# beer-asr/beer

Measured on AMD Instinct MI355X. Metric: frames/sec per VB iteration (E+M), higher is better.
Workload: dtype f32

## Files before the change

beer_amd/_hip.py:

```python

import ctypes
import os
import threading

import torch

_HERE = os.path.dirname(os.path.abspath(__file__))
LIB_PATH = os.environ.get('BEER_HIP_LIB') or os.path.join(_HERE, 'csrc', 'libbeer_hip.so')

F32, F64, I16 = 0, 1, 2
FULL, DIAG, ISO = 0, 1, 2
SEG = 8
MAX_HUBS = 4
COV_CODE = {'full': FULL, 'diagonal': DIAG, 'isotropic': ISO}
EINVAL = -100000


class HipUnavailable(RuntimeError):
    'Raised when the HIP extension or the GPU is missing (no CPU fallback).'


class HipError(RuntimeError):
    rc = None

# ... 274 lines not shown
    'beer_ng_from_natural': _from,
    'beer_ing_expected_stats': _four, 'beer_ing_log_norm': _four, 'beer_ing_natural': _four,
    'beer_ing_from_natural': _from,
    'beer_dirichlet_expected_stats': _dir, 'beer_dirichlet_log_norm': _dir,
    'beer_dirichlet_natural': _dir, 'beer_dirichlet_from_natural': _dir,
    'beer_dirichlet_log_weights': _dir,
    'beer_sb_transform_stats': [c_i, c_i, c_p, c_p, c_p, c_p],
    'beer_sb_log_weights': [c_i, c_i, c_p, c_p, c_p, c_p, c_p],
    'beer_sb_set_log_weights': [c_i, c_i, c_i, c_p, c_p, c_p, c_p],
    'beer_sb_set_transform_stats': [c_i, c_i, c_i, c_p, c_p, c_p, c_p],
    'beer_gamma_expected_stats': _gam, 'beer_gamma_log_norm': _gam,
    'beer_gamma_natural': _gam,
    'beer_gamma_from_natural': [c_i, c_i, c_p, c_p, c_p, c_p],
    'beer_kl_div': [c_i, c_i, c_i, c_p, c_p, c_p, c_p, c_p, c_p, c_p],
    'beer_natural_grad_step': [c_i, c_l, c_p, c_p, c_p, c_d, c_p, c_p],
    'beer_suffstats_expand': [c_i, c_i, c_l, c_i, c_p, c_p, c_p],
    'beer_mixtureset_estep': [c_i, c_i, c_l, c_i, c_i, c_i, c_p, c_p, c_p, c_p, c_d,
                              c_p, c_p, c_p, c_p, c_p, c_z, c_p],
    'beer_normal_accumulate': [c_i, c_i, c_l, c_i, c_i, c_i, c_p, c_p, c_p, c_p, c_p, c_z,
                               c_p],
    'beer_mixture_estep_packed': [c_i, c_l, c_i, c_i, c_p, c_p, c_p, c_p, c_p, c_p, c_p, c_z,
                                  c_p],
    'beer_normal_accumulate_packed': [c_i, c_l, c_i, c_i, c_p, c_p, c_p, c_p, c_z, c_p],
    'beer_mixtureset_estep_packed': [c_i, c_l, c_i, c_i, c_i, c_p, c_p, c_p, c_p, c_p, c_p, c_p,
                                     c_z, c_p],
    'beer_mixtureset_accumulate_packed': [c_i, c_l, c_i, c_i, c_i, c_p, c_p, c_p, c_p, c_p, c_z,
                                          c_p],
    'beer_unpack_resps': [c_l, c_i, c_p, c_p, c_p],
    'beer_mixtureset_accumulate_fused': [c_i, c_l, c_i, c_i, c_i, c_p, c_p, c_p, c_p, c_p, c_p,
                                         c_p, c_p, c_z, c_p],
# ... 286 lines not shown
```

beer_amd/csrc/estep_bf16.hip:

```cpp

#include <cstdlib>
#include <type_traits>
#include <utility>

#include "estep_mfma.h"
#include "estep_tiles.h"

namespace beer_mfma {

namespace {

typedef __bf16 bf8 __attribute__((ext_vector_type(8)));
typedef unsigned int u4 __attribute__((ext_vector_type(4)));
typedef float f32x2 __attribute__((ext_vector_type(2)));

template <int V> using ic = std::integral_constant<int, V>;
template <int... I, typename F>
__device__ __forceinline__ void static_for_impl(std::integer_sequence<int, I...>, F&& f) {
    (f(ic<I>{}), ...);
}
template <int N, typename F>
__device__ __forceinline__ void static_for(F&& f) {
    static_for_impl(std::make_integer_sequence<int, N>{}, static_cast<F&&>(f));
}
// ... 62 lines not shown
    const int a = t & 0xff, b = ((t >> 8) & 0xff) + e, sq = t >> 16;
    if (a == Dp && b - e == Dp) {
        *is_const = true;
        return 0.0;
    }
    if (k >= K) return 0.0;
    if (sq) return b < D ? -0.5 * (double)row[cov == BEER_ISO ? D : D + b] : 0.0;
    if (a < D) {
        if (b >= D || b < a) return 0.0;
        return b == a ? -0.5 * (double)row[D + a * D + a]
                      : -0.5 * ((double)row[D + a * D + b] + (double)row[D + b * D + a]);
    }
    return b < D ? (double)row[b] : 0.0;
}

__global__ __launch_bounds__(256) void const_max_kernel(int cov, int D, int K,
                                                        const float* __restrict__ E,
                                                        const float* __restrict__ logw,
                                                        float* __restrict__ c0) {
    __shared__ double red[8];
    const int Q = stats_dim(cov, D);
    double m = -1.0e300;
    for (int k = threadIdx.x; k < K; k += blockDim.x) {
        const double v = const_total(cov, D, E + (size_t)k * Q, logw ? (double)logw[k] : 0.0);
        if (v == v && v > m && v < 1.0e300) m = v;
    }
    m = block_max(m, red);
    if (threadIdx.x == 0) c0[0] = m > -1.0e300 ? (float)m : 0.f;
}

__global__ __launch_bounds__(256) void packx_kernel(int cov, int D, int K, int NT,
                                                    const float* __restrict__ E,
                                                    const float* __restrict__ logw,
                                                    unsigned short* __restrict__ P,
                                                    int* __restrict__ tab, int G, int Gp,
                                                    const float* __restrict__ c0, int lane_major) {
    extern __shared__ __attribute__((aligned(16))) char pack_lds[];
    const int nk = nk16_of(cov, D), nent = nk * 32;
    const int slot = blockIdx.x;
    const int k = slot % Gp < G ? (slot / Gp) * G + slot % Gp : K;
    const int chunk = slot / (NT * 16), kk = slot % (NT * 16);
    const int c = lane_major ? kk % NT : 4 * (kk / 64) + (kk % 4);
    const int i = lane_major ? kk / NT : (kk % 64) / 4;
    if (slot == 0)
        for (int s = threadIdx.x; s < (nk + 1) * 8; s += blockDim.x) tab[s] = slabx_entry(cov, D, s);
    const int Qs = stats_dim(cov, D);
    float* rowl = reinterpret_cast<float*>(pack_lds);
    if (k < K)
        for (int q = threadIdx.x; q < Qs; q += blockDim.x) rowl[q] = E[(size_t)k * Qs + q];
    __syncthreads();
    unsigned short* base = P + ((size_t)chunk * nk * NT) * (NP * 512);
    auto put = [&](int q, float v) {
// ... 2 lines not shown
        unsigned short p[3];
        split3_scalar(v, p);
        dst[0] = p[0];
        dst[512] = p[1];
        dst[1024] = p[2];
    };
    const int nslab = nslabx_of(cov, D);
    for (int q = threadIdx.x; q < nent; q += blockDim.x) {
        bool is_const;
        const double v = entry_value(cov, D, K, k, q / 4, q % 4, rowl, &is_const);
        if (!is_const) {
            put(q, (float)v);
        } else if (q % 4 == 0) {
            const bool last = q / 4 == nslab - 1;
            const double want = k < K ? const_share(cov, D, q / 4, rowl, logw ? (double)logw[k] : 0.0) -
                                            (last ? (double)c0[0] : 0.0)
                                      : (last ? kPadLogit : 0.0);
            const float hi = (float)want;
            const double rem = (want - (double)hi) * (1.0 / (double)kConstEps);
            put(q, hi);
            put(q + 1, (rem == rem && fabs(rem) < 1.0e30) ? (float)rem : 0.f);
            put(q + 2, 0.f);
            put(q + 3, 0.f);
        }
    }
}

inline int xcd_chunk_group(int ny, size_t chunk_bytes) {
    int cg = (int)((size_t)(2 << 20) / (chunk_bytes ? chunk_bytes : 1));
    return cg < 1 ? 1 : (cg > ny ? ny : cg);
}
// ... 1799 lines not shown
    const int Kreal = S * G, nk = nk16_of(cov, D);
    LlhxArgs a = {};
    a.nframes = nframes, a.D = D, a.K = S * f.Gp, a.S = S, a.G = f.Gp;
    a.gl = f.gl, a.jw = f.jw, a.nchunks = f.nchunks, a.nk = nk;
    a.nku = (nslabx_of(cov, D) + 7) / 8;
    a.X = X, a.resps = resps, a.log_norm = log_norm, a.llh_sum = llh_sum, a.img = image, a.s = s;
    const PtabLayout l = ptab_layout(f.nchunks, nk, f.NT);
    int* tab = reinterpret_cast<int*>(reinterpret_cast<char*>(ws) + l.tab);
    float* c0 = reinterpret_cast<float*>(reinterpret_cast<char*>(ws) + l.c0);
    a.P = ws, a.tab = tab, a.c0 = c0;
    if (f.xt) {
        a.xt_out = reinterpret_cast<float*>(reinterpret_cast<char*>(resps) +
                                            packed_tiles_bytes(nframes, a.K));
        a.xt_floats = xt_pieces(D) * (kPiece / 4);
    }
    hipLaunchKernelGGL(const_max_kernel, dim3(1), dim3(256), 0, s, cov, D, Kreal, expT, logw, c0);
    hipLaunchKernelGGL(packx_kernel, dim3(f.nchunks * f.NT * 16), dim3(256),
                       (size_t)stats_dim(cov, D) * sizeof(float), s, cov, D, Kreal, f.NT, expT, logw,
                       reinterpret_cast<unsigned short*>(ws), tab, G, f.Gp, c0,
                       f.lane_major ? 1 : 0);
    BEER_LAUNCH_CHECK();
    const int nku = f.lnfi ? f.nku : 0, gq = f.lnfi ? f.lnfi_g : f.GQ;
    for (const LlhxRow& r : kLlhxRows)
        if (r.NT == f.NT && r.GQ == gq && r.nku == nku && r.packed == f.packed && r.lno == f.lno &&
            r.img == f.img && r.bl == f.bl) {
            const auto launch = cov == BEER_FULL ? r.full : r.sq;
            return launch ? launch(a) : BEER_EINVAL;
        }
    return BEER_EINVAL;
}

// ... 87 lines not shown
    BEER_LAUNCH_CHECK();
    return BEER_OK;
}

}

int acc_bf16x3_packed(int cov, int64_t nframes, int D, int K, const float* X, const void* Rimg,
                      double* acc, void* ws, size_t ws_bytes, hipStream_t s, int S, int G,
                      const float* SR) {
    const AccxForm f = accx_form(cov, D, K, S, G, SR != nullptr);
    const AccxLayout l = accx_layout(cov, nframes, D, K, S, G, SR != nullptr);
    if (f.rc != BEER_OK || ws_bytes < l.bytes) return BEER_EINVAL;
    char* w = reinterpret_cast<char*>(ws);
    double* Sp = reinterpret_cast<double*>(w + l.Sp);
    int* tab = reinterpret_cast<int*>(w + l.tab);
    hipError_t e = hipMemsetAsync(Sp, 0, (size_t)K * f.nslab * 4 * sizeof(double), s);
    if (e != hipSuccess) return -(int)e;
    hipLaunchKernelGGL(tabx_kernel, dim3(1), dim3(256), 0, s, cov, D, f.nslab, tab);
    BEER_LAUNCH_CHECK();
    const int64_t tiles = (nframes + kAxFT - 1) / kAxFT;
    const float* Xt;
    if (f.xt_reused) {
        Xt = reinterpret_cast<const float*>(reinterpret_cast<const char*>(Rimg) +
                                            packed_tiles_bytes(nframes, K));
    } else {
        float* image = reinterpret_cast<float*>(w + l.Xt);
        hipLaunchKernelGGL(xt_image_kernel, dim3((unsigned)tiles), dim3(256), 0, s, nframes, D, f.NX,
                           X, image);
        BEER_LAUNCH_CHECK();
        Xt = image;
    }
    float* Gt = nullptr;
    if (f.sr) {
// ... 155 lines not shown
                     const float* sr, const void* image, double* acc, void* ws, size_t ws_bytes,
                     hipStream_t s) {
    const AccfForm f = accf_form(cov, D, S, G, image != nullptr);
    const AccfLayout l = accf_layout(cov, D, S, G);
    if (f.rc != BEER_OK || ws_bytes < l.bytes) return BEER_EINVAL;
    const int Kreal = S * G, K = S * f.Gp, NTC = f.NTC, nk = nk16_of(cov, D);
    const int nchunks = f.nchunks, kpad = nchunks * NTC * 16;
    const int nslab = nslab_of(cov, D), nq = nslab * 4;
    char* w = reinterpret_cast<char*>(ws);
    void* P = w + l.P;
    int* tab = reinterpret_cast<int*>(w + l.tab);
    float* c0 = reinterpret_cast<float*>(w + l.c0);
    double* Sp = reinterpret_cast<double*>(w + l.Sp);
    hipError_t e = hipMemsetAsync(Sp, 0, (size_t)Kreal * nq * sizeof(double), s);
    if (e != hipSuccess) return -(int)e;
    hipLaunchKernelGGL(const_max_kernel, dim3(1), dim3(256), 0, s, cov, D, Kreal, expT, logw, c0);
    hipLaunchKernelGGL(packx_kernel, dim3(kpad), dim3(256),
                       (size_t)stats_dim(cov, D) * sizeof(float), s, cov, D, Kreal, NTC, expT, logw,
                       reinterpret_cast<unsigned short*>(P), tab, G, f.Gp, c0, 0);
    BEER_LAUNCH_CHECK();
    const int waves = f.waves;
    const int rounds = beer::option(BEER_OPT_ACCF_ROUNDS);
    int64_t gz = ((waves == 8 ? 256 : 512) * rounds + nchunks - 1) / nchunks;
    gz = (gz + 7) / 8 * 8;
    const int64_t chain = nframes >= ((int64_t)4 << 20) ? kAfMaxFramesPerWave : kAfMaxFramesPerWave / 2;
    const int64_t min_z = (nframes + (int64_t)waves * chain - 1) / ((int64_t)waves * chain);
    const int64_t max_z = (nframes + 32 * waves - 1) / (32 * waves);
    if (gz > max_z) gz = max_z;
    if (gz < min_z) gz = min_z;
    if (gz < 1) gz = 1;
    const FrameSplit z = frame_split(nframes, gz, 32 * waves);
// ... 27 lines not shown
```

beer_amd/csrc/estep_tiles.h:

```cpp
#pragma once
#include <type_traits>

#include <hip/hip_runtime.h>

#include "common.h"

namespace beer_mfma {

using namespace beer;

typedef float f32x4 __attribute__((ext_vector_type(4)));
typedef double f64x4 __attribute__((ext_vector_type(4)));

template <typename T> struct Mma;
template <> struct Mma<float> {
    using acc_t = f32x4;
    using vec4_t = f32x4;
    static __device__ __forceinline__ acc_t mma(float a, float b, acc_t c) {
        return __builtin_amdgcn_mfma_f32_16x16x4f32(a, b, c, 0, 0, 0);
    }
    static __device__ __forceinline__ int row(int g, int r) { return 4 * g + r; }
    static __device__ __forceinline__ float exp_neg(float x) {
        return __builtin_amdgcn_exp2f(x * 1.44269504088896340736f);
    }
// ... 233 lines not shown
        acc[idx] += v;
    }
}
__global__ void unpack_kernel(int cov, int D, int K, const double* __restrict__ Sp,
                              double* __restrict__ acc) {
    unpack_stats<false>(cov, D, K, Sp, acc);
}
__global__ void unpackx_kernel(int cov, int D, int K, const double* __restrict__ Sp,
                               double* __restrict__ acc) {
    unpack_stats<true>(cov, D, K, Sp, acc);
}
__global__ void tabx_kernel(int cov, int D, int n, int* __restrict__ tab) {
    for (int s = blockIdx.x * blockDim.x + threadIdx.x; s < n; s += gridDim.x * blockDim.x)
        tab[s] = slabx_entry(cov, D, s);
}

}

constexpr int kPackedFrames = 64, kPackedComps = 128, kPackedPieces = 3;
constexpr int kPackedPlaneWords = kPackedComps * kPackedFrames / 2;

__host__ __device__ inline size_t packed_word(int64_t tau, int nblk, int beta, int kk, int f6) {
    const int half = kk * kPackedFrames + (((f6 >> 3) ^ (kk & 7)) << 3) + (f6 & 7);
    return ((size_t)tau * nblk + beta) * (kPackedPieces * kPackedPlaneWords) + (half >> 1);
}

__device__ __forceinline__ unsigned cvt_pk_bf16(float a, float b) {
    typedef __bf16 bf2_t __attribute__((ext_vector_type(2)));
    typedef float f2_t __attribute__((ext_vector_type(2)));
    const f2_t v = {a, b};
// ... 312 lines not shown
```

beer_amd/csrc/expfam.hip:

```cpp

#include "common.h"

using namespace beer;

namespace {

constexpr int kNwThreads = 1024;
inline int nw_threads(int K, int D) {
    return K <= 512 && D >= 16 ? 1024 : 256;
}
constexpr int kMaxFullDim = 128;




template <typename T>
__global__ __launch_bounds__(kNwThreads) void nw_expected_stats_kernel(
    int D, const T* __restrict__ mean, const T* __restrict__ scale,
    const T* __restrict__ W, const T* __restrict__ dof, T* __restrict__ out,
    T* __restrict__ lnorm) {
    extern __shared__ __attribute__((aligned(16))) char smem[];
    double* A = reinterpret_cast<double*>(smem);
    double* m = A + D * D;
    double* pm = m + D;
// ... 386 lines not shown
template <typename T>
__global__ __launch_bounds__(64) void kl_kernel(int Q, const T* es, const T* eq,
                                                const T* ep, const T* lq,
                                                const T* lp, T* out) {
    const int k = blockIdx.x;
    double s = 0.0;
    for (int i = threadIdx.x; i < Q; i += 64) {
        const size_t j = (size_t)k * Q + i;
        s += (double)es[j] * ((double)ep[j] - (double)eq[j]);
    }
    s = wave_sum(s);
    if (threadIdx.x == 0) out[k] = (T)((double)lp[k] - (double)lq[k] - s);
}

template <typename T>
__global__ void nat_grad_kernel(int64_t n, const T* ep, const T* eq, const T* st,
                                double lr, T* out) {
    const int64_t i = (int64_t)blockIdx.x * blockDim.x + threadIdx.x;
    if (i >= n) return;
    const double q = (double)eq[i];
    out[i] = (T)(q + lr * ((double)ep[i] + (double)st[i] - q));
}

template <typename T>
__global__ void suffstats_kernel(int cov, int64_t T_, int D, const T* X, T* out) {
    const int Q = stats_dim(cov, D);
    const int64_t total = T_ * Q;
    for (int64_t idx = (int64_t)blockIdx.x * blockDim.x + threadIdx.x; idx < total;
         idx += (int64_t)gridDim.x * blockDim.x) {
        const int64_t t = idx / Q;
        const int q = (int)(idx % Q);
        const T* x = X + t * D;
        T v;
        if (q < D) {
            v = x[q];
        } else if (q >= Q - 2) {
// ... 149 lines not shown
    return BEER_OK;
}

template <typename T>
int nat_grad_launch(int64_t n, const void* ep, const void* eq, const void* st, double lr,
                    void* out, void* stream) {
    BEER_REQUIRE(n >= 0);
    if (n == 0) return BEER_OK;
    hipLaunchKernelGGL(nat_grad_kernel<T>, dim3(blocks_for(n, 256)), dim3(256), 0,
                       as_stream(stream), n, (const T*)ep, (const T*)eq, (const T*)st, lr, (T*)out);
    BEER_LAUNCH_CHECK();
    return BEER_OK;
}

template <typename T>
int suffstats_launch(int cov, int64_t T_, int D, const void* X, void* out, void* stream) {
    BEER_REQUIRE(T_ >= 0 && D >= 1 && cov >= 0 && cov <= 2);
    if (T_ == 0) return BEER_OK;
    const int64_t total = T_ * stats_dim(cov, D);
    const int blocks = (int)((total + 255) / 256 > 65536 ? 65536 : (total + 255) / 256);
    hipLaunchKernelGGL(suffstats_kernel<T>, dim3(blocks), dim3(256), 0, as_stream(stream), cov, T_,
                       D, (const T*)X, (T*)out);
    BEER_LAUNCH_CHECK();
    return BEER_OK;
}

}


namespace {
// ... 292 lines not shown
}
int beer_gamma_log_norm(int dtype, int n, const void* shape, const void* rate, void* out, void* stream) {
    BEER_DISPATCH(dtype, gamma_launch, 3, n, shape, rate, out, nullptr, stream);
}

int beer_kl_div(int dtype, int K, int Q, const void* es, const void* eq, const void* ep,
                const void* lq, const void* lp, void* out, void* stream) {
    BEER_DISPATCH(dtype, kl_launch, K, Q, es, eq, ep, lq, lp, out, stream);
}

int beer_natural_grad_step(int dtype, int64_t n, const void* eta_prior, const void* eta_post,
                           const void* stats, double lrate, void* out, void* stream) {
    BEER_DISPATCH(dtype, nat_grad_launch, n, eta_prior, eta_post, stats, lrate, out, stream);
}

int beer_suffstats_expand(int dtype, int cov, int64_t T, int D, const void* X, void* out,
                          void* stream) {
    BEER_DISPATCH(dtype, suffstats_launch, cov, T, D, X, out, stream);
}

}
```

beer_amd/dists/families.py:

```python

import math

import torch

from .. import _hip
from ..stats import FrameStats, reference_layout_enabled
from .expfam import ConjugateLikelihood, ExponentialFamily, make_std_params

__all__ = [
    'NormalLikelihood', 'NormalWishart', 'NormalWishartStdParams',
    'NormalDiagonalLikelihood', 'NormalGamma', 'NormalGammaStdParams',
    'IsotropicNormalLikelihood', 'IsotropicNormalGamma',
    'IsotropicNormalGammaStdParams',
    'CategoricalLikelihood', 'Dirichlet', 'DirichletStdParams',
    'GammaLikelihood', 'Gamma', 'GammaStdParams',
]


def _run(name, dtype, ints, ins, outs):
    code = _hip.dtype_code(dtype)
    dins = [_hip.on_device(t, dtype) for t in ins]
    _hip.call(name, code, *ints, *[_hip.ptr(t) for t in dins], *[_hip.ptr(t) for t in outs])


# ... 352 lines not shown
    def log_weights(self):
        return self._memoised('logw', lambda: self._launch('beer_dirichlet_log_weights'))

    def log_weights64(self):
        c = self.params.concentrations
        if c.dtype == torch.float64:
            return self.log_weights()

        def compute():
            c2 = c.double().reshape(1, -1) if c.dim() <= 1 else c.double()
            out = _empty(tuple(c2.shape), c2, torch.float64)
            _run('beer_dirichlet_log_weights', torch.float64, tuple(c2.shape), (c2,), (out,))
            return out.to(c.device).view(c.shape)
        return self._memoised('logw64', compute)

    def expected_value(self):
        c = self.params.concentrations
        return c / c.sum(dim=-1, keepdim=True)



class GammaLikelihood(ConjugateLikelihood):
    def __init__(self, dim):
        self.dim = dim

    def sufficient_statistics_dim(self, zero_stats=True):
        return 2 * self.dim + (1 if zero_stats else 0)

    @staticmethod
    def sufficient_statistics(data):
# ... 64 lines not shown
```

beer_amd/inference/batch.py:

```python

import os
import threading

import torch

from .. import _hip, hmm_kernels as hk, kernels
from ..models.gaussians import NormalSet
from ..models.mixtures import Mixture, MixtureSet, TiedMixtureSet
from ..models.modelset import JointModelSet
from ..models.sequence import HMM, BigramPhoneLoop, PhoneLoop, unit_start_categories
from ..models.vae import VAE
from ..stats import FrameStats
from .objectives import EvidenceLowerBoundInstance

__all__ = ['accumulate_elbo', 'pack_utterances', 'decode_batch', 'sample_paths_batch',
           'log_evidence_batch', 'unit_starts_batch', 'unit_counts_batch',
           'unit_start_margins_batch', 'unit_segments_batch', 'ShardStatics',
           'decode_nbest_batch']

_SCRATCH_CAP = 48 << 30
_scratch_bytes = [int(os.environ['BEER_SCRATCH_GB']) << 30 if 'BEER_SCRATCH_GB' in os.environ
                  else None]


# ... 115 lines not shown


_KL_BESIDE = os.environ.get('BEER_KL_SIDE_STREAM', '1') != '0'


def _kl_beside_the_estep(model, device):
    if not _KL_BESIDE or isinstance(model, VAE) or device.type != 'cuda' or _capturing():
        return torch.as_tensor(model.kl_div_posterior_prior()), None
    main = torch.cuda.current_stream(device)
    for param in model.bayesian_parameters():
        for dist in (getattr(param, 'posterior', None), getattr(param, 'prior', None)):
            if dist is not None and hasattr(dist, 'expected_sufficient_statistics'):
                dist.expected_sufficient_statistics()
                dist.log_norm()
                dist.natural_parameters()
    side_streams = _local.__dict__.setdefault('side_streams', {})
    side = side_streams.get(device)
    if side is None:
        side = side_streams[device] = torch.cuda.Stream(device)
    side.wait_stream(main)
    with torch.cuda.stream(side):
        kl = torch.as_tensor(model.kl_div_posterior_prior())
        done = side.record_event()
    return kl, done


def _finish(model, value_terms, kl, nutt, acc, datasize, total_frames):
    value = value_terms - float(nutt) * kl.to(value_terms.device, torch.float64)
    return EvidenceLowerBoundInstance(value, acc, model.bayesian_parameters(),
                                      total_frames, datasize)


def _like(param, t):
    return t.to(dtype=param.stats.dtype, device=param.stats.device)


def _mixture_batch(model, X, lengths, datasize, labels, max_frames, statics=None):
    ns = model.normalset
    K, cov = len(ns), ns.cov_type
    dev, dtype = X.device, X.dtype
    exp_T = ns.means_precisions.natural_form()
    lw = model._log_weights().view(1, K)
    Q = FrameStats(X[:1], cov).shape[1]
    acc = torch.zeros(K, Q, dtype=torch.float64, device=dev)
    utt_llh = torch.zeros(len(lengths), dtype=torch.float64, device=dev)

    def offsets_and_scales():
        off = torch.zeros(len(lengths) + 1, dtype=torch.int64)
        off[1:] = torch.cumsum(torch.as_tensor(lengths, dtype=torch.int64), 0)
        up = _hip.upload({'off': off, 'scales': torch.as_tensor(
            [datasize / float(T) for T in lengths], dtype=torch.float64)}, dev)
        return off, up['off'], up['scales']
    statics = statics if statics is not None else ShardStatics()
    statics.bind(lengths)
    skey = ('mixture', len(lengths), float(datasize), str(dev))
    off, off_dev, scales = statics.entry(skey, 'offsets', offsets_and_scales)
    lab_dev = None if labels is None else \
        _hip.on_device(torch.as_tensor(labels)).to(torch.int64).contiguous()
    if lab_dev is not None and model.nested:
        M = len(model.modelset)
        lw_sets = model.modelset.leaf_log_weights()
    for run in _sub_batches(lengths, K * X.element_size(), max_frames):
        done = _throttle()
        f0, f1 = int(off[run[0]]), int(off[run[-1] + 1])
        stats = FrameStats(X[f0:f1], cov)
        lab = None if lab_dev is None else lab_dev[f0:f1]
        wide = kernels.wide_mixture_split(stats, K, cov) if lab is None else None
        seg = off_dev[run[0]:run[-1] + 2] - f0
        if lab is not None and model.nested:
            set_norm, resps = kernels.mixtureset_estep(stats, exp_T, lw_sets, M, K // M, cov)
            onehot = torch.zeros_like(set_norm).scatter_(1, lab.view(-1, 1), 1.)
            hk.segment_sum(kernels.rowdot(set_norm, onehot), seg, len(run),
                           out=utt_llh[run[0]:run[-1] + 1])
            kernels.normal_accumulate(stats, resps, onehot, M, K // M, cov, acc=acc)
            done.record()
            continue
        if lab is None and kernels.packed_path_ok(stats, K, cov):
            log_norm, resps = kernels.mixture_estep_packed(stats, exp_T, lw, K, cov)
        elif wide:
            log_norm, resps = kernels.wide_mixture_estep(stats, exp_T, lw, K, cov, wide)
        else:
            log_norm, resps = kernels.mixtureset_estep(stats, exp_T, lw, 1, K, cov, labels=lab)
        hk.segment_sum(log_norm.view(-1), seg, len(run), out=utt_llh[run[0]:run[-1] + 1])
        kernels.normal_accumulate(stats, resps, None, K, 1, cov, acc=acc)
        done.record()
    value_terms = (scales * utt_llh).sum()
    out = {**model._weights_accumulate(acc), ns.means_precisions: _like(ns.means_precisions, acc)}
    return value_terms, out


def _emission_estep(groups, stats, dtype, for_accumulate=False):
    cols, comps = [], []
    for grp, S, G in groups:
        ns = _normalset(grp)
        gstats = stats.as_cov(ns.cov_type)
        if isinstance(grp, TiedMixtureSet):
            tied = grp.estep(gstats)
            cols.append(tied[2])
            comps.append(('tied',) + tied)
            continue
        lw = grp.leaf_log_weights() if isinstance(grp, MixtureSet) else None
# ... 469 lines not shown
```

beer_amd/inference/captured.py:

```python

import warnings

import torch

from .. import _hip
from .objectives import evidence_lower_bound
from .optimizers import VBConjugateOptimizer

__all__ = ['CapturedIteration']


def _drop_memos(params):
    for p in params:
        p.posterior.__dict__['_memo'] = {}
        p.__dict__.pop('_kl_memo', None)


class CapturedIteration:

    def __init__(self, model, optim, data, datasize=-1, **kwargs):
        if not isinstance(optim, VBConjugateOptimizer):
            raise TypeError('CapturedIteration drives a VBConjugateOptimizer')
        self.model, self.optim = model, optim
        self.lengths = None
        if isinstance(data, tuple) and len(data) == 2 and isinstance(data[0], torch.Tensor):
            from ..stats import FrameImages
            from .batch import ShardStatics
            self.data, self.lengths = _hip.on_device(data[0]), [int(n) for n in data[1]]
            kwargs.setdefault('statics', ShardStatics())
            if 'frame_images' not in kwargs and self.data.dtype == torch.float32:
# ... 64 lines not shown
            return self._eager()
        if entry is not None and not self._same(entry['signature'], self._signature()):
            self._entries = {t: None for t in self._entries}
            entry = None
        if entry is None:
            entry = self._capture(turn, members)
            if entry is None:
                return self._eager()
            self.mode = 'captured'
        else:
            self.mode = 'replayed'
        entry['graph'].replay()
        optim.update_count += 1
        every = [p for group in optim.groups for p in group]
        _drop_memos(every)
        for p, st in zip(members, entry['stats']):
            p.stats = st
        return entry['value']

    def _capture(self, turn, members):
        optim = self.optim
        every = [p for group in optim.groups for p in group]
        if not all(VBConjugateOptimizer._capturable(group) for group in optim.groups) or \
                not all(t.is_cuda for p in every for t in p.posterior._tensors()):
            self._all_eager = True
            return None
        homes = [p.posterior.params for p in members]
        home_tensors = [tuple(p.posterior._tensors()) for p in members]
        count, use_graph = optim.update_count, optim.graph
        _drop_memos(every)
        torch.cuda.synchronize()
        graph = torch.cuda.CUDAGraph()
        try:
            optim.graph = False
            with torch.cuda.graph(graph, capture_error_mode='thread_local'):
                elbo = self._iteration()
                value = elbo.value
                dsts = [dst for old in home_tensors for dst in old]
                srcs = [src for p in members for src in p.posterior._tensors()]
                torch._foreach_copy_(dsts, srcs)
        except RuntimeError as err:
            refused = not isinstance(err, _hip.HipError) or isinstance(err, _hip.HipInvalid) \
                or 900 <= -(err.rc or 0) <= 908
            if not refused:
                raise
            self._all_eager = True
            warnings.warn(f'CapturedIteration: the iteration could not be recorded as a HIP graph '
                          f'({type(err).__name__}: {err}); it runs eagerly', RuntimeWarning)
            return None
        finally:
            optim.graph, optim.update_count = use_graph, count
            for p, params in zip(members, homes):
                p.posterior.params = params
            _drop_memos(every)
        entry = {'graph': graph, 'value': value, 'stats': [p.stats for p in members],
                 'signature': self._signature()}
        self._entries[turn] = entry
        return entry
```

beer_amd/inference/objectives.py:

```python

import threading

import torch

from .. import _hip
from ..hmm_kernels import check_sample, segment_sum

__all__ = ['evidence_lower_bound', 'EvidenceLowerBoundInstance']


def add_acc_stats(acc_stats1, acc_stats2):
    out = dict(acc_stats1)
    for key, val in acc_stats2.items():
        out[key] = out[key] + val if key in out else val
    return out


def scale_acc_stats(acc_stats, scale):
    return {key: scale * val for key, val in acc_stats.items()}


class EvidenceLowerBoundInstance:

    def __init__(self, value, acc_stats, model_parameters, minibatchsize, datasize):
# ... 16 lines not shown
        if self._datasize != other._datasize:
            raise ValueError('Cannot add ELBOs evaluated on different data set')
        return EvidenceLowerBoundInstance(
            self.value + other.value,
            add_acc_stats(self._acc_stats, other._acc_stats),
            self._model_parameters.union(other._model_parameters),
            self._minibatchsize + other._minibatchsize,
            self._datasize)

    def backward(self, std_params=True):
        if std_params and isinstance(self.value, torch.Tensor) and self.value.requires_grad:
            (-self.value).backward()
        scale = self._datasize / self._minibatchsize
        for parameter in self._model_parameters:
            try:
                parameter.store_stats(scale * self._acc_stats[parameter])
            except KeyError:
                pass

    def sync(self, model):
        self._model_parameters = set(model.bayesian_parameters())


_span_lock = threading.Lock()
_spans = {}


def _span(n, device):
    key = (device, n)
    with _span_lock:
        off = _spans.get(key)
        if off is None:
            if len(_spans) >= 64:
# ... 36 lines not shown
```

beer_amd/inference/optimizers.py:

```python

import os
import pickle
import warnings

import torch

from .. import _hip

__all__ = ['VBConjugateOptimizer', 'VBOptimizer']

_STATE = ('lrate', 'update_count')


class VBConjugateOptimizer:

    _warned = False

    def __init__(self, groups, lrate=1., graph=None):
        self.groups = [list(members) for members in groups]
        self.lrate, self.update_count = lrate, 0
        self.graph = (os.environ.get('BEER_MSTEP_GRAPH', '1') != '0') if graph is None \
            else bool(graph)
        self._captured = {}

# ... 57 lines not shown
            return False
        if entry is not None and (entry[4] != self.lrate or entry[5] != self._signature(members)):
            entry = None
        if entry is None:
            if not self._capturable(members):
                self._captured[key] = False
                return False
            statics = [p.stats.detach().clone() for p in members]
            etas = [p.posterior.natural_parameters().detach().clone() for p in members]
            torch.cuda.synchronize()
            graph = torch.cuda.CUDAGraph()
            try:
                with torch.cuda.graph(graph, capture_error_mode='thread_local'):
                    for p, st, eta in zip(members, statics, etas):
                        p.stats = st
                        eta.copy_(p.natural_grad_update(self.lrate, eta_q=eta))
            except RuntimeError as err:
                refused = not isinstance(err, _hip.HipError) or isinstance(err, _hip.HipInvalid) \
                    or 900 <= -(err.rc or 0) <= 908
                for p, st in zip(members, statics):
                    p.stats = st
                    p.posterior.__dict__.pop('_memo', None)
                    p.__dict__.pop('_kl_memo', None)
                if not refused or os.environ.get('BEER_MSTEP_GRAPH_STRICT') == '1':
                    raise
                self._captured[key] = False
                if not VBConjugateOptimizer._warned:
                    VBConjugateOptimizer._warned = True
                    warnings.warn(f'VBConjugateOptimizer: the M-step of group {key} could not be '
                                  f'captured as a HIP graph ({type(err).__name__}: {err}); this '
                                  'group takes the eager update from here on', RuntimeWarning)
# ... 49 lines not shown
```

beer_amd/models/parameters.py:

```python

import uuid

import torch

from .. import _hip
from ..dists import kl_div

__all__ = ['ParameterRef', 'BayesianParameter', 'ConjugateBayesianParameter']


class ParameterRef:
    __slots__ = ('uuid',)

    def __init__(self, uuid):
        self.uuid = uuid

    def __hash__(self):
        return hash(self.uuid)

    def __eq__(self, other):
        return getattr(other, 'uuid', None) == self.uuid

    def __getstate__(self):
        return {'uuid': self.uuid}
# ... 84 lines not shown
        self.register_buffer('stats', init_stats.clone().detach())
        if likelihood_fn is None:
            likelihood_fn = prior.conjugate()
        self.likelihood_fn = likelihood_fn

    def __len__(self):
        return 1 if self.stats.dim() <= 1 else self.stats.shape[0]

    def __getitem__(self, key):
        return self.__class__(prior=self.prior[key], posterior=self.posterior[key],
                              init_stats=self.stats[key], likelihood_fn=self.likelihood_fn)

    def zero_stats(self):
        self.stats.zero_()

    def store_stats(self, acc_stats):
        self.stats = acc_stats.clone().detach() if acc_stats.requires_grad else acc_stats

    def natural_form(self):
        return self.posterior.expected_sufficient_statistics()

    def natural_grad_update(self, lrate, eta_q=None):
        self.dispatch(before_update=True)
        eta_p = self.prior.natural_parameters()
        if eta_q is None:
            eta_q = self.posterior.natural_parameters()
        home, dtype = eta_q.device, eta_q.dtype
        dp, dq = _hip.on_device(eta_p, dtype), _hip.on_device(eta_q)
        ds = _hip.on_device(self.stats, dtype)
        if ds.shape != dq.shape:
            raise ValueError(f'statistics {tuple(ds.shape)} do not match the natural '
                             f'parameters {tuple(dq.shape)}')
        new = torch.empty_like(dq)
        _hip.call('beer_natural_grad_step', _hip.dtype_code(dtype), dq.numel(),
                  _hip.ptr(dp), _hip.ptr(dq), _hip.ptr(ds), float(lrate), _hip.ptr(new))
        self.posterior.update_from_natural_parameters(new.to(home))
        self.dispatch(before_update=False)
        return new
```

include/beer_hip.h:

```cpp
#ifndef BEER_HIP_H
#define BEER_HIP_H

#include <stddef.h>
#include <stdint.h>

#ifdef __cplusplus
extern "C" {
#endif

#define BEER_F32 0
#define BEER_F64 1
#define BEER_I16 2

#define BEER_FULL 0
#define BEER_DIAG 1
#define BEER_ISO 2

#define BEER_OK 0
#define BEER_EINVAL (-100000)

int beer_hip_version(void);
int beer_hip_device_count(void);

#define BEER_OPT_AX_MAXFRAMES 0
// ... 77 lines not shown
                              const void* rate, void* out, void* stream);
int beer_gamma_log_norm(int dtype, int n, const void* shape, const void* rate,
                        void* out , void* stream);
int beer_gamma_natural(int dtype, int n, const void* shape, const void* rate,
                       void* out, void* stream);
int beer_gamma_from_natural(int dtype, int n, const void* eta, void* shape,
                            void* rate, void* stream);

int beer_kl_div(int dtype, int K, int Q, const void* exp_stats_q,
                const void* eta_q, const void* eta_p, const void* lnorm_q,
                const void* lnorm_p, void* out, void* stream);

int beer_natural_grad_step(int dtype, int64_t n, const void* eta_prior,
                           const void* eta_post, const void* stats,
                           double lrate, void* out, void* stream);

int beer_suffstats_expand(int dtype, int cov, int64_t T, int D, const void* X,
                          void* out, void* stream);


int beer_mixtureset_estep(int dtype, int cov, int64_t T, int D, int S, int G,
                          const void* X, const void* exp_stats,
                          const void* log_weights, const int64_t* labels,
                          double stat_scale, void* pc_llh, void* log_norm,
                          void* comp_resps, double* llh_sum, void* workspace,
                          size_t workspace_bytes, void* stream);

size_t beer_estep_workspace_bytes(int dtype, int cov, int D, int S, int G);
size_t beer_accumulate_workspace_bytes(int dtype, int cov, int D, int S, int G);
size_t beer_accumulate_frames_workspace_bytes(int dtype, int cov, int64_t T, int D, int S, int G);
// ... 519 lines not shown
```

Baseline: 269.9 million.

## Cut launches and host work in the VB update and E-step paths

The const-max reduction is folded into every packx block, so its separate single-block launch goes away, and the table build is merged with zeroing of the partial sums in one kernel instead of a memset. New fused kernels handle scaling stats into place and the Dirichlet posterior update (concentrations, expected stats, log weights, log norm) in one launch, and the natural-gradient step can run in place. Per-utterance segment sums run on a side stream, segment offsets are cached, and captured graphs keep posterior memos across replays. The cost is redundant const-max work in each packx block and more complex memo and stream bookkeeping.

```diff
diff --git a/beer_amd/_hip.py b/beer_amd/_hip.py
--- a/beer_amd/_hip.py
+++ b/beer_amd/_hip.py
@@ -312,6 +312,8 @@
     'beer_gamma_from_natural': [c_i, c_i, c_p, c_p, c_p, c_p],
     'beer_kl_div': [c_i, c_i, c_i, c_p, c_p, c_p, c_p, c_p, c_p, c_p],
     'beer_natural_grad_step': [c_i, c_l, c_p, c_p, c_p, c_d, c_p, c_p],
+    'beer_stats_natural_step': [c_i, c_i, c_l, c_p, c_d, c_p, c_p, c_d, c_p, c_p, c_p],
+    'beer_dirichlet_update': [c_i, c_i, c_i, c_p, c_p, c_p, c_p, c_p, c_p],
     'beer_suffstats_expand': [c_i, c_i, c_l, c_i, c_p, c_p, c_p],
     'beer_mixtureset_estep': [c_i, c_i, c_l, c_i, c_i, c_i, c_p, c_p, c_p, c_p, c_d,
                               c_p, c_p, c_p, c_p, c_p, c_z, c_p],
diff --git a/beer_amd/csrc/estep_bf16.hip b/beer_amd/csrc/estep_bf16.hip
--- a/beer_amd/csrc/estep_bf16.hip
+++ b/beer_amd/csrc/estep_bf16.hip
@@ -100,11 +100,8 @@
     return b < D ? (double)row[b] : 0.0;
 }
 
-__global__ __launch_bounds__(256) void const_max_kernel(int cov, int D, int K,
-                                                        const float* __restrict__ E,
-                                                        const float* __restrict__ logw,
-                                                        float* __restrict__ c0) {
-    __shared__ double red[8];
+__device__ inline float const_max(int cov, int D, int K, const float* __restrict__ E,
+                                  const float* __restrict__ logw, double* red) {
     const int Q = stats_dim(cov, D);
     double m = -1.0e300;
     for (int k = threadIdx.x; k < K; k += blockDim.x) {
@@ -112,7 +109,7 @@
         if (v == v && v > m && v < 1.0e300) m = v;
     }
     m = block_max(m, red);
-    if (threadIdx.x == 0) c0[0] = m > -1.0e300 ? (float)m : 0.f;
+    return m > -1.0e300 ? (float)m : 0.f;
 }
 
 __global__ __launch_bounds__(256) void packx_kernel(int cov, int D, int K, int NT,
@@ -120,8 +117,11 @@
                                                     const float* __restrict__ logw,
                                                     unsigned short* __restrict__ P,
                                                     int* __restrict__ tab, int G, int Gp,
-                                                    const float* __restrict__ c0, int lane_major) {
+                                                    float* __restrict__ c0, int lane_major) {
     extern __shared__ __attribute__((aligned(16))) char pack_lds[];
+    __shared__ double red[8];
+    const float c0v = const_max(cov, D, K, E, logw, red);
+    if (blockIdx.x == 0 && threadIdx.x == 0) c0[0] = c0v;
     const int nk = nk16_of(cov, D), nent = nk * 32;
     const int slot = blockIdx.x;
     const int k = slot % Gp < G ? (slot / Gp) * G + slot % Gp : K;
@@ -154,7 +154,7 @@
         } else if (q % 4 == 0) {
             const bool last = q / 4 == nslab - 1;
             const double want = k < K ? const_share(cov, D, q / 4, rowl, logw ? (double)logw[k] : 0.0) -
-                                            (last ? (double)c0[0] : 0.0)
+                                            (last ? (double)c0v : 0.0)
                                       : (last ? kPadLogit : 0.0);
             const float hi = (float)want;
             const double rem = (want - (double)hi) * (1.0 / (double)kConstEps);
@@ -1984,7 +1984,6 @@
                                             packed_tiles_bytes(nframes, a.K));
         a.xt_floats = xt_pieces(D) * (kPiece / 4);
     }
-    hipLaunchKernelGGL(const_max_kernel, dim3(1), dim3(256), 0, s, cov, D, Kreal, expT, logw, c0);
     hipLaunchKernelGGL(packx_kernel, dim3(f.nchunks * f.NT * 16), dim3(256),
                        (size_t)stats_dim(cov, D) * sizeof(float), s, cov, D, Kreal, f.NT, expT, logw,
                        reinterpret_cast<unsigned short*>(ws), tab, G, f.Gp, c0,
@@ -2102,9 +2101,10 @@
     char* w = reinterpret_cast<char*>(ws);
     double* Sp = reinterpret_cast<double*>(w + l.Sp);
     int* tab = reinterpret_cast<int*>(w + l.tab);
-    hipError_t e = hipMemsetAsync(Sp, 0, (size_t)K * f.nslab * 4 * sizeof(double), s);
-    if (e != hipSuccess) return -(int)e;
-    hipLaunchKernelGGL(tabx_kernel, dim3(1), dim3(256), 0, s, cov, D, f.nslab, tab);
+    const int64_t nsums = (int64_t)K * f.nslab * 4;
+    const int64_t zblocks = (nsums + 255) / 256;
+    hipLaunchKernelGGL(tabx_zero_kernel, dim3((unsigned)(zblocks < 2048 ? zblocks : 2048)),
+                       dim3(256), 0, s, cov, D, f.nslab, tab, Sp, nsums);
     BEER_LAUNCH_CHECK();
     const int64_t tiles = (nframes + kAxFT - 1) / kAxFT;
     const float* Xt;
@@ -2290,7 +2290,6 @@
     double* Sp = reinterpret_cast<double*>(w + l.Sp);
     hipError_t e = hipMemsetAsync(Sp, 0, (size_t)Kreal * nq * sizeof(double), s);
     if (e != hipSuccess) return -(int)e;
-    hipLaunchKernelGGL(const_max_kernel, dim3(1), dim3(256), 0, s, cov, D, Kreal, expT, logw, c0);
     hipLaunchKernelGGL(packx_kernel, dim3(kpad), dim3(256),
                        (size_t)stats_dim(cov, D) * sizeof(float), s, cov, D, Kreal, NTC, expT, logw,
                        reinterpret_cast<unsigned short*>(P), tab, G, f.Gp, c0, 0);
diff --git a/beer_amd/csrc/estep_tiles.h b/beer_amd/csrc/estep_tiles.h
--- a/beer_amd/csrc/estep_tiles.h
+++ b/beer_amd/csrc/estep_tiles.h
@@ -271,6 +271,13 @@
     for (int s = blockIdx.x * blockDim.x + threadIdx.x; s < n; s += gridDim.x * blockDim.x)
         tab[s] = slabx_entry(cov, D, s);
 }
+__global__ void tabx_zero_kernel(int cov, int D, int n, int* __restrict__ tab,
+                                 double* __restrict__ Sp, int64_t count) {
+    const int64_t first = (int64_t)blockIdx.x * blockDim.x + threadIdx.x;
+    const int64_t stride = (int64_t)gridDim.x * blockDim.x;
+    for (int64_t s = first; s < n; s += stride) tab[s] = slabx_entry(cov, D, (int)s);
+    for (int64_t i = first; i < count; i += stride) Sp[i] = 0.0;
+}
 
 }
 
diff --git a/beer_amd/csrc/expfam.hip b/beer_amd/csrc/expfam.hip
--- a/beer_amd/csrc/expfam.hip
+++ b/beer_amd/csrc/expfam.hip
@@ -424,12 +424,68 @@
 }
 
 template <typename T>
+__device__ __forceinline__ T nat_grad_value(T ep, T eq, T st, double lr) {
+    const double q = (double)eq;
+    return (T)(q + lr * ((double)ep + (double)st - q));
+}
+
+template <typename T>
 __global__ void nat_grad_kernel(int64_t n, const T* ep, const T* eq, const T* st,
                                 double lr, T* out) {
     const int64_t i = (int64_t)blockIdx.x * blockDim.x + threadIdx.x;
     if (i >= n) return;
-    const double q = (double)eq[i];
-    out[i] = (T)(q + lr * ((double)ep[i] + (double)st[i] - q));
+    out[i] = nat_grad_value<T>(ep[i], eq[i], st[i], lr);
+}
+
+template <typename T>
+__device__ __forceinline__ T handoff_value(double a, T scale) {
+#pragma clang fp contract(off)
+    const T v = (T)a;
+    return v * scale;
+}
+
+template <typename T, typename SRC>
+__global__ void stats_step_kernel(int64_t n, const SRC* acc, T scale, const T* ep, const T* eq,
+                                  double lr, T* stats, T* out) {
+    const int64_t i = (int64_t)blockIdx.x * blockDim.x + threadIdx.x;
+    if (i >= n) return;
+    const T st = handoff_value<T>((double)acc[i], scale);
+    stats[i] = st;
+    if (out) out[i] = nat_grad_value<T>(ep[i], eq[i], st, lr);
+}
+
+template <typename T>
+__global__ __launch_bounds__(64) void dirichlet_update_kernel(int S, int G, const T* eta, T* conc,
+                                                              T* exp_stats, T* log_w,
+                                                              T* log_norm) {
+    const int s = blockIdx.x, lane = threadIdx.x;
+    const T* e = eta + (size_t)s * G;
+    double part = 0.0;
+    for (int g = lane; g < G - 1; g += 64) part += (double)e[g];
+    const double eta_tot = wave_sum(part);
+    const T c_last = (T)((double)e[G - 1] - eta_tot + 1.0);
+    auto c_of = [&](int g) { return g < G - 1 ? (T)((double)e[g] + 1.0) : c_last; };
+    double tot = 0.0, lg = 0.0;
+    for (int g = lane; g < G; g += 64) {
+        const T c = c_of(g);
+        conc[(size_t)s * G + g] = c;
+        tot += (double)c;
+        lg += lgamma((double)c);
+    }
+    tot = wave_sum(tot);
+    lg = wave_sum(lg);
+    if (lane == 0) log_norm[s] = (T)(lg - lgamma(tot));
+    const double psi_last = digamma((double)c_last);
+    const double last = psi_last - digamma(tot);
+    for (int g = lane; g < G - 1; g += 64) {
+        const double v = digamma((double)c_of(g)) - psi_last;
+        exp_stats[(size_t)s * G + g] = (T)v;
+        log_w[(size_t)s * G + g] = (T)(v + last);
+    }
+    if (lane == 0) {
+        exp_stats[(size_t)s * G + G - 1] = (T)last;
+        log_w[(size_t)s * G + G - 1] = (T)last;
+    }
 }
 
 template <typename T>
@@ -609,6 +665,37 @@
 }
 
 template <typename T>
+int stats_step_launch(int acc_dtype, int64_t n, const void* acc, double scale, const void* ep,
+                      const void* eq, double lr, void* stats, void* out, void* stream) {
+    const bool wide = acc_dtype == BEER_F64;
+    BEER_REQUIRE(n >= 0 && (wide || acc_dtype == (sizeof(T) == 4 ? BEER_F32 : BEER_F64)));
+    if (n == 0) return BEER_OK;
+    BEER_REQUIRE(acc && stats && (!out || (ep && eq)));
+    const dim3 g(blocks_for(n, 256)), b(256);
+    if (wide)
+        hipLaunchKernelGGL((stats_step_kernel<T, double>), g, b, 0, as_stream(stream), n,
+                           (const double*)acc, (T)scale, (const T*)ep, (const T*)eq, lr, (T*)stats,
+                           (T*)out);
+    else
+        hipLaunchKernelGGL((stats_step_kernel<T, T>), g, b, 0, as_stream(stream), n, (const T*)acc,
+                           (T)scale, (const T*)ep, (const T*)eq, lr, (T*)stats, (T*)out);
+    BEER_LAUNCH_CHECK();
+    return BEER_OK;
+}
+
+template <typename T>
+int dirichlet_update_launch(int S, int G, const void* eta, void* conc, void* exp_stats,
+                            void* log_w, void* log_norm, void* stream) {
+    BEER_REQUIRE(S >= 0 && G >= 1);
+    if (S == 0) return BEER_OK;
+    BEER_REQUIRE(eta && conc && exp_stats && log_w && log_norm);
+    hipLaunchKernelGGL(dirichlet_update_kernel<T>, dim3(S), dim3(64), 0, as_stream(stream), S, G,
+                       (const T*)eta, (T*)conc, (T*)exp_stats, (T*)log_w, (T*)log_norm);
+    BEER_LAUNCH_CHECK();
+    return BEER_OK;
+}
+
+template <typename T>
 int suffstats_launch(int cov, int64_t T_, int D, const void* X, void* out, void* stream) {
     BEER_REQUIRE(T_ >= 0 && D >= 1 && cov >= 0 && cov <= 2);
     if (T_ == 0) return BEER_OK;
@@ -931,6 +1018,19 @@
     BEER_DISPATCH(dtype, nat_grad_launch, n, eta_prior, eta_post, stats, lrate, out, stream);
 }
 
+int beer_stats_natural_step(int dtype, int acc_dtype, int64_t n, const void* acc, double scale,
+                            const void* eta_prior, const void* eta_post, double lrate,
+                            void* stats, void* eta_out, void* stream) {
+    BEER_DISPATCH(dtype, stats_step_launch, acc_dtype, n, acc, scale, eta_prior, eta_post, lrate,
+                  stats, eta_out, stream);
+}
+
+int beer_dirichlet_update(int dtype, int S, int G, const void* eta, void* conc, void* exp_stats,
+                          void* log_weights, void* log_norm, void* stream) {
+    BEER_DISPATCH(dtype, dirichlet_update_launch, S, G, eta, conc, exp_stats, log_weights,
+                  log_norm, stream);
+}
+
 int beer_suffstats_expand(int dtype, int cov, int64_t T, int D, const void* X, void* out,
                           void* stream) {
     BEER_DISPATCH(dtype, suffstats_launch, cov, T, D, X, out, stream);
diff --git a/beer_amd/dists/families.py b/beer_amd/dists/families.py
--- a/beer_amd/dists/families.py
+++ b/beer_amd/dists/families.py
@@ -5,7 +5,7 @@
 
 from .. import _hip
 from ..stats import FrameStats, reference_layout_enabled
-from .expfam import ConjugateLikelihood, ExponentialFamily, make_std_params
+from .expfam import ConjugateLikelihood, ExponentialFamily, ParametersView, make_std_params
 
 __all__ = [
     'NormalLikelihood', 'NormalWishart', 'NormalWishartStdParams',
@@ -390,6 +390,29 @@
             return out.to(c.device).view(c.shape)
         return self._memoised('logw64', compute)
 
+    def update_from_natural_parameters(self, natural_params):
+        eta = natural_params.detach()
+        if isinstance(self.params, ParametersView) or eta.dim() not in (1, 2) or \
+                eta.dtype not in (torch.float32, torch.float64):
+            return super().update_from_natural_parameters(natural_params)
+        single = eta.dim() == 1
+        home, dtype = eta.device, eta.dtype
+        deta = _hip.on_device(eta.view(1, -1) if single else eta)
+        S, G = deta.shape
+        new = lambda *shape: torch.empty(*shape, dtype=dtype, device=deta.device)
+        conc, exp, logw, lnorm = new(S, G), new(S, G), new(S, G), new(S)
+        _hip.call('beer_dirichlet_update', _hip.dtype_code(dtype), S, G, _hip.ptr(deta),
+                  _hip.ptr(conc), _hip.ptr(exp), _hip.ptr(logw), _hip.ptr(lnorm))
+        conc, exp, logw, lnorm = (t.to(home) for t in (conc, exp, logw, lnorm))
+        if single:
+            conc, exp, logw, lnorm = conc.view(-1), exp.view(-1), logw.view(-1), lnorm[0]
+        self.params = type(self.params)(conc)
+        self.__dict__['_memo'] = {}
+        self._memoised('nat', lambda: eta)
+        self._memoised('exp', lambda: exp)
+        self._memoised('logw', lambda: logw)
+        self._memoised('lnorm', lambda: lnorm)
+
     def expected_value(self):
         c = self.params.concentrations
         return c / c.sum(dim=-1, keepdim=True)
diff --git a/beer_amd/inference/batch.py b/beer_amd/inference/batch.py
--- a/beer_amd/inference/batch.py
+++ b/beer_amd/inference/batch.py
@@ -153,15 +153,20 @@
                 dist.expected_sufficient_statistics()
                 dist.log_norm()
                 dist.natural_parameters()
-    side_streams = _local.__dict__.setdefault('side_streams', {})
-    side = side_streams.get(device)
-    if side is None:
-        side = side_streams[device] = torch.cuda.Stream(device)
+    side = _side_stream(device)
     side.wait_stream(main)
     with torch.cuda.stream(side):
         kl = torch.as_tensor(model.kl_div_posterior_prior())
         done = side.record_event()
     return kl, done
+
+
+def _side_stream(device):
+    side_streams = _local.__dict__.setdefault('side_streams', {})
+    side = side_streams.get(device)
+    if side is None:
+        side = side_streams[device] = torch.cuda.Stream(device)
+    return side
 
 
 def _finish(model, value_terms, kl, nutt, acc, datasize, total_frames):
@@ -182,7 +187,13 @@
     lw = model._log_weights().view(1, K)
     Q = FrameStats(X[:1], cov).shape[1]
     acc = torch.zeros(K, Q, dtype=torch.float64, device=dev)
-    utt_llh = torch.zeros(len(lengths), dtype=torch.float64, device=dev)
+    main = side = None
+    if _KL_BESIDE and labels is None and dev.type == 'cuda' and not _capturing():
+        main, side = torch.cuda.current_stream(dev), _side_stream(dev)
+        side.wait_stream(main)
+    held = []
+    with torch.cuda.stream(side):
+        utt_llh = torch.zeros(len(lengths), dtype=torch.float64, device=dev)
 
     def offsets_and_scales():
         off = torch.zeros(len(lengths) + 1, dtype=torch.int64)
@@ -205,7 +216,8 @@
         stats = FrameStats(X[f0:f1], cov)
         lab = None if lab_dev is None else lab_dev[f0:f1]
         wide = kernels.wide_mixture_split(stats, K, cov) if lab is None else None
-        seg = off_dev[run[0]:run[-1] + 2] - f0
+        seg = statics.entry(skey, ('seg', run[0], run[-1]),
+                            lambda: off_dev[run[0]:run[-1] + 2] - f0)
         if lab is not None and model.nested:
             set_norm, resps = kernels.mixtureset_estep(stats, exp_T, lw_sets, M, K // M, cov)
             onehot = torch.zeros_like(set_norm).scatter_(1, lab.view(-1, 1), 1.)
@@ -220,10 +232,18 @@
             log_norm, resps = kernels.wide_mixture_estep(stats, exp_T, lw, K, cov, wide)
         else:
             log_norm, resps = kernels.mixtureset_estep(stats, exp_T, lw, 1, K, cov, labels=lab)
-        hk.segment_sum(log_norm.view(-1), seg, len(run), out=utt_llh[run[0]:run[-1] + 1])
+        if side is not None:
+            side.wait_event(main.record_event())
+            held.append(log_norm)
+        with torch.cuda.stream(side):
+            hk.segment_sum(log_norm.view(-1), seg, len(run), out=utt_llh[run[0]:run[-1] + 1])
         kernels.normal_accumulate(stats, resps, None, K, 1, cov, acc=acc)
         done.record()
-    value_terms = (scales * utt_llh).sum()
+    with torch.cuda.stream(side):
+        value_terms = (scales * utt_llh).sum()
+    if side is not None:
+        main.wait_event(side.record_event())
+    del held
     out = {**model._weights_accumulate(acc), ns.means_precisions: _like(ns.means_precisions, acc)}
     return value_terms, out
 
diff --git a/beer_amd/inference/captured.py b/beer_amd/inference/captured.py
--- a/beer_amd/inference/captured.py
+++ b/beer_amd/inference/captured.py
@@ -14,6 +14,24 @@
     for p in params:
         p.posterior.__dict__['_memo'] = {}
         p.__dict__.pop('_kl_memo', None)
+
+
+_KEPT = ('nat', 'exp', 'lnorm', 'logw')
+
+
+def _valid_memo(post, keys):
+    tensors = post._tensors()
+    sig = tuple(t._version for t in tensors)
+    return {key: hit for key, hit in post.__dict__.get('_memo', {}).items()
+            if key in keys and len(hit[0]) == len(tensors) and hit[1] == sig and
+            all(a is b for a, b in zip(hit[0], tensors)) and
+            isinstance(hit[2], torch.Tensor) and hit[2].is_cuda}
+
+
+def _rekey(post, kept):
+    tensors = post._tensors()
+    sig = tuple(t._version for t in tensors)
+    post.__dict__['_memo'] = {key: (tensors, sig, hit[2]) for key, hit in kept.items()}
 
 
 class CapturedIteration:
@@ -108,11 +126,12 @@
         optim.update_count += 1
         every = [p for group in optim.groups for p in group]
         _drop_memos(every)
-        for p, st in zip(members, entry['stats']):
+        for p, st, kept in zip(members, entry['stats'], entry['kept']):
             p.stats = st
+            _rekey(p.posterior, kept)
         return entry['value']
 
-    def _capture(self, turn, members):
+    def _capture(self, turn, members, keys=_KEPT):
         optim = self.optim
         every = [p for group in optim.groups for p in group]
         if not all(VBConjugateOptimizer._capturable(group) for group in optim.groups) or \
@@ -122,7 +141,11 @@
         homes = [p.posterior.params for p in members]
         home_tensors = [tuple(p.posterior._tensors()) for p in members]
         count, use_graph = optim.update_count, optim.graph
+        kepts = [_valid_memo(p.posterior, keys) for p in members]
         _drop_memos(every)
+        for p, kept in zip(members, kepts):
+            _rekey(p.posterior, kept)
+        produced = None
         torch.cuda.synchronize()
         graph = torch.cuda.CUDAGraph()
         try:
@@ -132,6 +155,14 @@
                 value = elbo.value
                 dsts = [dst for old in home_tensors for dst in old]
                 srcs = [src for p in members for src in p.posterior._tensors()]
+                news = [_valid_memo(p.posterior, keys) for p in members]
+                produced = [key for key in keys if all(
+                    key not in kept or (key in new and new[key][2].shape == kept[key][2].shape and
+                                        new[key][2].dtype == kept[key][2].dtype)
+                    for kept, new in zip(kepts, news))]
+                if len(produced) == len(keys):
+                    dsts += [kept[key][2] for kept in kepts for key in kept]
+                    srcs += [new[key][2] for kept, new in zip(kepts, news) for key in kept]
                 torch._foreach_copy_(dsts, srcs)
         except RuntimeError as err:
             refused = not isinstance(err, _hip.HipError) or isinstance(err, _hip.HipInvalid) \
@@ -147,7 +178,12 @@
             for p, params in zip(members, homes):
                 p.posterior.params = params
             _drop_memos(every)
+            for p, kept in zip(members, kepts):
+                _rekey(p.posterior, kept)
+        if len(produced) < len(keys):
+            del graph
+            return self._capture(turn, members, tuple(produced))
         entry = {'graph': graph, 'value': value, 'stats': [p.stats for p in members],
-                 'signature': self._signature()}
+                 'kept': kepts, 'signature': self._signature()}
         self._entries[turn] = entry
         return entry
diff --git a/beer_amd/inference/objectives.py b/beer_amd/inference/objectives.py
--- a/beer_amd/inference/objectives.py
+++ b/beer_amd/inference/objectives.py
@@ -54,9 +54,13 @@
         scale = self._datasize / self._minibatchsize
         for parameter in self._model_parameters:
             try:
-                parameter.store_stats(scale * self._acc_stats[parameter])
+                acc = self._acc_stats[parameter]
             except KeyError:
-                pass
+                continue
+            if hasattr(parameter, 'natural_grad_update') and not isinstance(scale, torch.Tensor):
+                parameter.store_stats(acc, scale)
+            else:
+                parameter.store_stats(scale * acc)
 
     def sync(self, model):
         self._model_parameters = set(model.bayesian_parameters())
diff --git a/beer_amd/inference/optimizers.py b/beer_amd/inference/optimizers.py
--- a/beer_amd/inference/optimizers.py
+++ b/beer_amd/inference/optimizers.py
@@ -95,7 +95,9 @@
                 with torch.cuda.graph(graph, capture_error_mode='thread_local'):
                     for p, st, eta in zip(members, statics, etas):
                         p.stats = st
-                        eta.copy_(p.natural_grad_update(self.lrate, eta_q=eta))
+                        new = p.natural_grad_update(self.lrate, eta_q=eta, in_place=True)
+                        if new is not eta:
+                            eta.copy_(new)
             except RuntimeError as err:
                 refused = not isinstance(err, _hip.HipError) or isinstance(err, _hip.HipInvalid) \
                     or 900 <= -(err.rc or 0) <= 908
diff --git a/beer_amd/models/parameters.py b/beer_amd/models/parameters.py
--- a/beer_amd/models/parameters.py
+++ b/beer_amd/models/parameters.py
@@ -122,13 +122,28 @@
     def zero_stats(self):
         self.stats.zero_()
 
-    def store_stats(self, acc_stats):
+    def store_stats(self, acc_stats, scale=None):
+        stats = self.stats
+        if scale is not None and \
+                isinstance(acc_stats, torch.Tensor) and acc_stats.is_cuda and stats.is_cuda and \
+                not acc_stats.requires_grad and acc_stats.device == stats.device and \
+                acc_stats.shape == stats.shape and stats.is_contiguous() and \
+                stats.dtype in (torch.float32, torch.float64) and \
+                acc_stats.dtype in (stats.dtype, torch.float64) and \
+                acc_stats.untyped_storage().data_ptr() != stats.untyped_storage().data_ptr():
+            src = acc_stats.contiguous()
+            _hip.call('beer_stats_natural_step', _hip.dtype_code(stats.dtype),
+                      _hip.dtype_code(src.dtype), src.numel(), _hip.ptr(src), float(scale), None,
+                      None, 0., _hip.ptr(stats), None)
+            return
+        if scale is not None:
+            acc_stats = scale * acc_stats
         self.stats = acc_stats.clone().detach() if acc_stats.requires_grad else acc_stats
 
     def natural_form(self):
         return self.posterior.expected_sufficient_statistics()
 
-    def natural_grad_update(self, lrate, eta_q=None):
+    def natural_grad_update(self, lrate, eta_q=None, in_place=False):
         self.dispatch(before_update=True)
         eta_p = self.prior.natural_parameters()
         if eta_q is None:
@@ -139,7 +154,7 @@
         if ds.shape != dq.shape:
             raise ValueError(f'statistics {tuple(ds.shape)} do not match the natural '
                              f'parameters {tuple(dq.shape)}')
-        new = torch.empty_like(dq)
+        new = dq if in_place and dq is eta_q else torch.empty_like(dq)
         _hip.call('beer_natural_grad_step', _hip.dtype_code(dtype), dq.numel(),
                   _hip.ptr(dp), _hip.ptr(dq), _hip.ptr(ds), float(lrate), _hip.ptr(new))
         self.posterior.update_from_natural_parameters(new.to(home))
diff --git a/include/beer_hip.h b/include/beer_hip.h
--- a/include/beer_hip.h
+++ b/include/beer_hip.h
@@ -115,6 +115,14 @@
 int beer_natural_grad_step(int dtype, int64_t n, const void* eta_prior,
                            const void* eta_post, const void* stats,
                            double lrate, void* out, void* stream);
+
+int beer_stats_natural_step(int dtype, int acc_dtype, int64_t n, const void* acc,
+                            double scale, const void* eta_prior, const void* eta_post,
+                            double lrate, void* stats, void* eta_out, void* stream);
+
+int beer_dirichlet_update(int dtype, int S, int G, const void* eta, void* conc,
+                          void* exp_stats, void* log_weights, void* log_norm,
+                          void* stream);
 
 int beer_suffstats_expand(int dtype, int cov, int64_t T, int D, const void* X,
                           void* out, void* stream);
```

Result: slower. 266.4 million (-1.3%).
